# JanEGerken/HEAL-SWIN

Hardware: AMD Instinct MI355X
Metric: images/sec fwd+bwd, HEAL-SWIN nside=256 seg, batch=8 at 1/2/4/8 MI355X (higher is better)
Workload: dtype bf16

## Files before the change

### heal_swin_amd/csrc/expand_ln_head.hip

```cpp
#include "ln_head_device.h"
#include "hs_depth_loss.h"

#pragma clang fp contract(off)
#include "hs_depth_target.h"
#include "hs_depth_metrics.h"
#pragma clang fp contract(fast)

namespace hs {
namespace {

constexpr int kP = 4;
constexpr int kRowB = 256;
constexpr int kPatchRow = 128;

constexpr int kHistBins = kKP * kKP;

__device__ __forceinline__ int argmax_merge(float best, int arg, float ob, int oa) {
    const bool n0 = best != best, n1 = ob != ob;
    const int lower = arg < oa ? arg : oa;
    if (n0 || n1) return n0 && n1 ? lower : (n0 ? arg : oa);
    return best > ob ? arg : (ob > best ? oa : lower);
}

struct TailLane {
    float num = 0.f, den = 0.f;
    uint32_t pred4 = 0;
    uint32_t bad_rows = 0;
    uint32_t* hist = nullptr;
    float4 m4, lv4;
    double dsum[depth_metrics::kNSums];
};

struct TailCe {
    const uint8_t* labels;
    const float* class_w;
    float* loss_part;
    int n_classes;
    __device__ __forceinline__ bool has_loss() const { return labels != nullptr; }
    __device__ __forceinline__ bool ce_row(TailLane& st, const f32x16& lg, const float (&bk)[8], int64_t orow, bool live, int half,
                                           float (&v)[8], int& yl) const {
        if (!labels) return false;
        float m = -INFINITY;
#pragma unroll
        for (int r = 0; r < 8; ++r) {
            v[r] = lg[r] + bk[r];
            if (class_natural(r, half) < n_classes) m = fmaxf(m, v[r]);
        }
        m = fmaxf(m, __shfl_xor(m, 32, 64));
        yl = live ? (int)labels[orow] : 255;
        float ssum = 0.f, pick = 0.f;
#pragma unroll
        for (int r = 0; r < 8; ++r) {
            const int cls = class_natural(r, half);
            if (cls < n_classes) ssum += __builtin_amdgcn_exp2f((v[r] - m) * kLog2e);
            pick = cls == yl ? v[r] : pick;
        }
        ssum += __shfl_xor(ssum, 32, 64);
        pick += __shfl_xor(pick, 32, 64);
        const float wy = yl < n_classes ? (class_w ? class_w[yl] : 1.f) : 0.f;
        if (half == 0) {
            st.num = fmaf(wy, m + __builtin_amdgcn_logf(ssum) * kLn2 - pick, st.num);
            st.den += wy;
        }
        return true;
    }
    __device__ __forceinline__ void row(TailLane& st, const f32x16& lg, const float (&bk)[8], int64_t orow, int, bool live,
                                        int lane) const {
        float v[8];
        int yl;
        ce_row(st, lg, bk, orow, live, lane >> 5, v, yl);
    }
};

struct TailCeStep : TailCe {
    uint8_t* preds;
    unsigned long long* conf;
    unsigned long long* bad;
    __device__ __forceinline__ bool has_loss() const { return true; }
    __device__ __forceinline__ void row(TailLane& st, const f32x16& lg, const float (&bk)[8], int64_t orow, int p, bool live,
                                        int lane) const {
        const int half = lane >> 5;
        float v[8];
        int yl;
        if (!ce_row(st, lg, bk, orow, live, half, v, yl)) return;
        float best = -INFINITY;
        int arg = 4 * half < n_classes ? 4 * half : 64;
#pragma unroll
        for (int r = 0; r < 8; ++r) {
            const int cls = class_natural(r, half);
            if (cls < n_classes && !(best != best) && (v[r] > best || v[r] != v[r])) {
                best = v[r];
                arg = cls;
            }
        }
        const int pred = argmax_merge(best, arg, __shfl_xor(best, 32, 64), __shfl_xor(arg, 32, 64));
        st.pred4 |= (uint32_t)pred << (8 * p);
        if (conf) {
            const bool mine = live && half == 0;
            const int bin = mine && yl < n_classes ? yl * n_classes + pred : -1;
            st.bad_rows += (uint32_t)__popcll(__ballot(mine && yl >= n_classes));
            const int lead = __builtin_amdgcn_readfirstlane(bin);
            const unsigned long long same = __ballot(bin == lead);
            if (bin == lead) {
                if (lead >= 0 && lane == __ffsll((long long)same) - 1) atomicAdd(&st.hist[lead], (uint32_t)__popcll(same));
            } else if (bin >= 0) {
                atomicAdd(&st.hist[bin], 1u);
            }
        }
    }
};

struct TailDepth {
    const float* target;
    float* loss_part;
    int kind;
    float delta;
    __device__ __forceinline__ bool has_loss() const { return true; }
    __device__ __forceinline__ float depth_row(TailLane& st, const f32x16& lg, const float (&bk)[8], int64_t orow, bool live,
                                               int half) const {
        const float t = live && half == 0 ? target[orow] : INFINITY;
        if (depth_keep(t)) {
            st.num += depth_term(kind, delta, lg[0] + bk[0], lg[1] + bk[1], t);
            st.den += 1.f;
        }
        return t;
    }
    __device__ __forceinline__ void row(TailLane& st, const f32x16& lg, const float (&bk)[8], int64_t orow, int, bool live,
                                        int lane) const {
        depth_row(st, lg, bk, orow, live, lane >> 5);
    }
};

struct TailDepthStep : TailDepth {
    int n_out;
    TargetOp inv;
    depth_metrics::Rule rule;
    double* partial;
    float* preds;
    float* logvar_out;
    int64_t rows;
    __device__ __forceinline__ void row(TailLane& st, const f32x16& lg, const float (&bk)[8], int64_t orow, int p, bool live,
                                        int lane) const {
        const int half = lane >> 5;
        const float p0 = lg[0] + bk[0], p1 = lg[1] + bk[1], t = depth_row(st, lg, bk, orow, live, half);
        if (partial || preds) {
#pragma clang fp contract(off)
            const float m = target_op(p0, inv);
            if (partial && live && half == 0)
                depth_metrics::accumulate<float, float>(st.dsum, rule, m, target_op(t, inv), [&] { return p1; });
            st.m4.x = p == 0 ? m : st.m4.x;
            st.m4.y = p == 1 ? m : st.m4.y;
            st.m4.z = p == 2 ? m : st.m4.z;
            st.m4.w = p == 3 ? m : st.m4.w;
        }
        st.lv4.x = p == 0 ? p1 : st.lv4.x;
        st.lv4.y = p == 1 ? p1 : st.lv4.y;
        st.lv4.z = p == 2 ? p1 : st.lv4.z;
        st.lv4.w = p == 3 ? p1 : st.lv4.w;
    }
};

template <int NB, typename Loss>
__global__ void __launch_bounds__(256, 1) expand_ln_head_fwd_kernel(const uint16_t* __restrict__ xn, const uint16_t* __restrict__ xn_lo,
                                                                    const uint16_t* __restrict__ wexp,
                                                                    const uint16_t* __restrict__ wfold, const float* __restrict__ bvec,
                                                                    uint16_t* __restrict__ y, float* __restrict__ logits,
                                                                    float* __restrict__ mean_out, float* __restrict__ rstd_out,
                                                                    int64_t tokens, Loss ce) {
    constexpr bool kStep = std::is_same<Loss, TailCeStep>::value, kDStep = std::is_same<Loss, TailDepthStep>::value;
    constexpr int C = 32 * NB, KS = 2 * NB, NCH = C / 8;
    extern __shared__ __attribute__((aligned(16))) unsigned char smem[];
    unsigned char* wl = smem;
    unsigned char* patch = smem + kP * C * kRowB + (threadIdx.x >> 6) * (32 * kPatchRow);
    const int tid = threadIdx.x, lane = tid & 63, l31 = lane & 31, half = lane >> 5;

    for (int q = tid; q < kP * C * NCH; q += 256) {
        const int row = q / NCH, ch = q % NCH;
        *(uint4*)(wl + row * kRowB + ((ch ^ (row & 15)) << 4)) = *(const uint4*)(wexp + (int64_t)row * C + ch * 8);
    }
    bf16x8 wfa[NB][2], wfl[NB][2];
#pragma unroll
    for (int ct = 0; ct < NB; ++ct)
#pragma unroll
        for (int j = 0; j < 2; ++j) {
            const uint16_t* src = wfold + l31 * C + 32 * ct + 16 * j + 4 * half;
            const uint2 a = *(const uint2*)src, b = *(const uint2*)(src + 8);
            wfa[ct][j] = __builtin_bit_cast(bf16x8, make_uint4(a.x, a.y, b.x, b.y));
            const uint2 al = *(const uint2*)(src + 32 * C), bl = *(const uint2*)(src + 32 * C + 8);
            wfl[ct][j] = __builtin_bit_cast(bf16x8, make_uint4(al.x, al.y, bl.x, bl.y));
        }
    float bk[8];
    load_head_bias(bvec, half, bk);
    uint32_t* hist = (uint32_t*)(smem + kP * C * kRowB + 4 * 32 * kPatchRow);
    TailLane st;
    st.hist = hist + (tid >> 6) * kHistBins;
    if constexpr (kStep) {
        for (int j = tid; j < 4 * kHistBins; j += 256) hist[j] = 0;
    }
    if constexpr (kDStep) {
#pragma unroll
        for (int k = 0; k < depth_metrics::kNSums; ++k) st.dsum[k] = 0.0;
    }
    __syncthreads();

    const int sx = l31 & 15;
    const int64_t wave = (int64_t)blockIdx.x * 4 + (tid >> 6), nwaves = (int64_t)gridDim.x * 4;
    for (int64_t tok0 = wave * 32; tok0 < tokens; tok0 += nwaves * 32) {
        const int64_t tok = tok0 + l31;
        const bool live = tok < tokens;
        bf16x8 xb[KS];
#pragma unroll
        for (int ks = 0; ks < KS; ++ks) {
            const uint4 v = live ? *(const uint4*)(xn + tok * C + 16 * ks + 8 * half) : make_uint4(0, 0, 0, 0);
            xb[ks] = __builtin_bit_cast(bf16x8, v);
        }
        st.pred4 = 0;
        st.m4 = st.lv4 = make_float4(0.f, 0.f, 0.f, 0.f);
#pragma unroll 1
        for (int p = 0; p < kP; ++p) {
            f32x16 acc[NB];
#pragma unroll
            for (int ct = 0; ct < NB; ++ct)
#pragma unroll
                for (int r = 0; r < 16; ++r) acc[ct][r] = 0.f;
            const unsigned char* wrow = wl + (p * C + l31) * kRowB;
#pragma unroll
            for (int ks = 0; ks < KS; ++ks) {
                const int co = ((2 * ks + half) ^ sx) << 4;
#pragma unroll
                for (int ct = 0; ct < NB; ++ct) {
                    const bf16x8 a = *(const bf16x8*)(wrow + ct * 32 * kRowB + co);
                    acc[ct] = __builtin_amdgcn_mfma_f32_32x32x16_bf16(a, xb[ks], acc[ct], 0, 0, 0);
                }
            }
            if (xn_lo) {
#pragma unroll
                for (int ks = 0; ks < KS; ++ks) {
                    const uint4 v = live ? *(const uint4*)(xn_lo + tok * C + 16 * ks + 8 * half) : make_uint4(0, 0, 0, 0);
                    const int co = ((2 * ks + half) ^ sx) << 4;
#pragma unroll
                    for (int ct = 0; ct < NB; ++ct) {
                        const bf16x8 a = *(const bf16x8*)(wrow + ct * 32 * kRowB + co);
                        acc[ct] = __builtin_amdgcn_mfma_f32_32x32x16_bf16(a, __builtin_bit_cast(bf16x8, v), acc[ct], 0, 0, 0);
                    }
                }
            }
            const int64_t orow = tok * kP + p;
            if (y) {
#pragma unroll
                for (int pr = 0; pr < (NB + 1) / 2; ++pr) {
#pragma unroll
                    for (int t = 0; t < 2; ++t) {
                        const int ct = 2 * pr + t;
                        if (ct < NB) {
#pragma unroll
                            for (int g = 0; g < 4; ++g) {
                                const int chunk = 4 * t + g;
                                *(uint2*)(patch + l31 * kPatchRow + ((chunk ^ (l31 & 7)) << 4) + 8 * half) =
                                    make_uint2(pack_bf16x2(acc[ct][4 * g], acc[ct][4 * g + 1]), pack_bf16x2(acc[ct][4 * g + 2], acc[ct][4 * g + 3]));
                            }
                        }
                    }
                    __builtin_amdgcn_fence(__ATOMIC_RELEASE, "wavefront");
                    __builtin_amdgcn_wave_barrier();
                    constexpr int kChunksLast = (NB % 2) ? 4 : 8;
                    const int nchunks = (2 * pr + 1 < NB) ? 8 : kChunksLast;
#pragma unroll
                    for (int i = 0; i < 4; ++i) {
                        const int q = lane + 64 * i, row = q >> 3, chunk = q & 7;
                        const uint4 v = *(const uint4*)(patch + row * kPatchRow + ((chunk ^ (row & 7)) << 4));
                        if (chunk < nchunks && tok0 + row < tokens)
                            *(uint4*)(y + ((tok0 + row) * kP + p) * C + 64 * pr + chunk * 8) = v;
                    }
                    __builtin_amdgcn_fence(__ATOMIC_ACQUIRE, "wavefront");
                    __builtin_amdgcn_wave_barrier();
                }
            }
            float mean, rstd;
            row_stats<16>(acc, mean, rstd);
            f32x16 lg;
#pragma unroll
            for (int r = 0; r < 16; ++r) lg[r] = 0.f;
#pragma unroll
            for (int ct = 0; ct < NB; ++ct)
#pragma unroll
                for (int j = 0; j < 2; ++j) {
                    float xh[8];
#pragma unroll
                    for (int i = 0; i < 8; ++i) xh[i] = acc[ct][8 * j + i] * rstd;
                    lg = head_step<3>(lg, xh, wfa[ct][j], wfl[ct][j]);
                }
            ce.row(st, lg, bk, orow, p, live, lane);
            if (live) {
                if (logits) {
                    *(float4*)(logits + orow * kKP + 4 * half) = make_float4(lg[0] + bk[0], lg[1] + bk[1], lg[2] + bk[2], lg[3] + bk[3]);
                    *(float4*)(logits + orow * kKP + 8 + 4 * half) = make_float4(lg[4] + bk[4], lg[5] + bk[5], lg[6] + bk[6], lg[7] + bk[7]);
                }
                if (half == 0 && mean_out) {
                    mean_out[orow] = mean;
                    rstd_out[orow] = rstd;
                }
            }
        }
        if constexpr (kStep) {
            if (ce.preds && live && half == 0) *(uint32_t*)(ce.preds + tok * kP) = st.pred4;
        }
        if constexpr (kDStep) {
            if (live && half == 0) {
                if (ce.preds) *(float4*)(ce.preds + tok * kP) = st.m4;
                float* lv = ce.preds ? (ce.n_out > 1 ? ce.preds + ce.rows : nullptr) : ce.logvar_out;
                if (lv) *(float4*)(lv + tok * kP) = st.lv4;
            }
        }
    }
    if constexpr (kDStep) {
        if (ce.partial) {
            constexpr int NS = depth_metrics::kNSums;
            static_assert(NS * 256 * sizeof(double) <= kP * 64 * kRowB + 4 * 32 * kPatchRow, "lane sums must fit the LDS at C = 64");
            double* red = (double*)smem;
            __syncthreads();
#pragma unroll
            for (int k = 0; k < NS; ++k) red[k * 256 + tid] = st.dsum[k];
            __syncthreads();
            for (int h = 128; h > 0; h >>= 1) {
                for (int q = tid; q < NS * h; q += 256) {
                    const int k = q / h, j = q - k * h;
                    red[k * 256 + j] += red[k * 256 + j + h];
                }
                __syncthreads();
            }
            if (tid < NS) ce.partial[(int64_t)blockIdx.x * NS + tid] = red[tid * 256];
        }
    }
    if constexpr (kStep) {
        if (ce.conf) {
            __syncthreads();
            const int bins = ce.n_classes * ce.n_classes;
            if (tid < bins) {
                const uint32_t n = hist[tid] + hist[kHistBins + tid] + hist[2 * kHistBins + tid] + hist[3 * kHistBins + tid];
                if (n) atomicAdd(&ce.conf[tid], (unsigned long long)n);
            }
            if (lane == 0 && st.bad_rows) atomicAdd(&ce.bad[0], (unsigned long long)st.bad_rows);
        }
    }
    if (ce.has_loss()) {
        const float n = wave_sum(st.num), d = wave_sum(st.den);
        if (lane == 0) {
            ce.loss_part[2 * wave] = n;
            ce.loss_part[2 * wave + 1] = d;
        }
    }
}

}
}

extern "C" {

int hs_expand_ln_head_supported(int width, int children, int n_classes, int dtype) {
    return dtype == HS_BF16 && children == hs::kP && width % 32 == 0 && width >= 64 && width <= 128 && n_classes >= 1 && n_classes <= 16;
}

extern "C++" {
namespace {
template <typename Loss>
int launch_expand_ln_head(const void* xn, const void* xn_lo, const void* wexp, const void* wfold, const float* bvec, void* y, float* logits,
                          float* mean, float* rstd, int64_t tokens, int width, int children, int dtype, void* stream, Loss ce,
                          const char* who) {
    using namespace hs;
    HS_CHECK_ARG(xn && wexp && wfold && bvec, "%s: null pointer", who);
    HS_CHECK_ARG(tokens > 0, "%s: bad shape", who);
    HS_CHECK_ARG((y == nullptr) == (mean == nullptr) && (mean == nullptr) == (rstd == nullptr),
                 "%s: y, mean and rstd (what the backward needs) go together", who);
    if (!hs_expand_ln_head_supported(width, children, 1, dtype))
        return fail(HS_ERR_UNSUPPORTED, "%s: bf16, 4 children, C in {64, 96, 128} (got C = %d, children %d): the expand "
                    "weight must fit the LDS", who, width, children);
    HS_CHECK_ALIGNED(who, 16, xn, xn_lo, wexp, wfold, bvec, y);
    constexpr bool kStep = std::is_same<Loss, TailCeStep>::value;
    const size_t smem = (size_t)kP * width * kRowB + 4 * 32 * kPatchRow + (kStep ? 4 * kHistBins * sizeof(uint32_t) : 0);
    HS_CHECK_ARG(smem <= 160 * 1024, "%s: %zu bytes of LDS", who, smem);
    const dim3 grid((unsigned)hs_expand_ln_head_blocks(tokens)), block(256);
    if constexpr (kStep) {
        const int64_t groups = (tokens + 31) / 32, waves = (int64_t)grid.x * 4;
        HS_CHECK_ARG((groups + waves - 1) / waves < (1ll << 25), "%s: %lld tokens on %lld waves overflow the 32-bit histogram bins", who,
                     (long long)tokens, (long long)waves);
    }
    return with_width_blocks<4>(width, [&](auto nb) {
        auto kern = expand_ln_head_fwd_kernel<decltype(nb)::value, Loss>;
        static bool configured = false;
        if (!configured) {
            HS_HIP_CHECK(hipFuncSetAttribute((const void*)kern, hipFuncAttributeMaxDynamicSharedMemorySize, (int)smem));
            configured = true;
        }
        hipLaunchKernelGGL(kern, grid, block, smem, (hipStream_t)stream, (const uint16_t*)xn, (const uint16_t*)xn_lo,
                           (const uint16_t*)wexp, (const uint16_t*)wfold, bvec, (uint16_t*)y, logits, mean, rstd, tokens, ce);
        HS_LAUNCH_CHECK("expand_ln_head_fwd");
        return (int)HS_OK;
    });
}
int check_ce_loss(const char* who, const void* labels, const void* loss_partials, int n_classes) {
    HS_CHECK_ARG(labels && loss_partials, "%s: null pointer", who);
    return hs::check_class_count(who, n_classes);
}
int check_depth_loss(const char* who, const void* target, const void* loss_partials, int kind, float huber_delta, int n_out) {
    HS_CHECK_ARG(target && loss_partials, "%s: null pointer", who);
    return hs::check_depth_head(who, kind, huber_delta, n_out);
}
}
}

int64_t hs_expand_ln_head_blocks(int64_t tokens) {
    int64_t blocks = (tokens + 127) / 128;
    const int cus = hs::usable_cus();
    if (blocks > cus) blocks = cus;
    return blocks < 1 ? 1 : blocks;
}

int hs_expand_ln_head_fwd(const void* xn, const void* xn_lo, const void* wexp, const void* wfold, const float* bvec, void* y, float* logits,
                          float* mean, float* rstd, int64_t tokens, int width, int children, int dtype, void* stream) {
    HS_CHECK_ARG(logits, "hs_expand_ln_head_fwd: null pointer");
    return launch_expand_ln_head(xn, xn_lo, wexp, wfold, bvec, y, logits, mean, rstd, tokens, width, children, dtype, stream,
                                 hs::TailCe{nullptr, nullptr, nullptr, 0}, "hs_expand_ln_head_fwd");
}

int hs_expand_ln_head_ce_fwd(const void* xn, const void* xn_lo, const void* wexp, const void* wfold, const float* bvec, const uint8_t* labels,
                             const float* class_weights, int n_classes, void* y, float* logits, float* mean, float* rstd,
                             float* loss_partials, int64_t tokens, int width, int children, int dtype, void* stream) {
    if (int e = check_ce_loss("hs_expand_ln_head_ce_fwd", labels, loss_partials, n_classes)) return e;
    return launch_expand_ln_head(xn, xn_lo, wexp, wfold, bvec, y, logits, mean, rstd, tokens, width, children, dtype, stream,
                                 hs::TailCe{labels, class_weights, loss_partials, n_classes}, "hs_expand_ln_head_ce_fwd");
}

int hs_expand_ln_head_ce_step_fwd(const void* xn, const void* xn_lo, const void* wexp, const void* wfold, const float* bvec,
                                  const uint8_t* labels, const float* class_weights, int n_classes, void* y, float* logits, float* mean,
                                  float* rstd, float* loss_partials, uint8_t* preds, int64_t* confmat, int64_t* bad, int64_t tokens,
                                  int width, int children, int dtype, void* stream) {
    const char* who = "hs_expand_ln_head_ce_step_fwd";
    if (int e = check_ce_loss(who, labels, loss_partials, n_classes)) return e;
    HS_CHECK_ARG(!confmat || bad, "%s: confmat needs bad (the counter of labels >= n_classes)", who);
    HS_CHECK_ARG(((uintptr_t)preds & 3) == 0, "%s: preds must be 4-byte aligned", who);
    return launch_expand_ln_head(xn, xn_lo, wexp, wfold, bvec, y, logits, mean, rstd, tokens, width, children, dtype, stream,
                                 hs::TailCeStep{{labels, class_weights, loss_partials, n_classes}, preds, (unsigned long long*)confmat,
                                                (unsigned long long*)bad}, who);
}

int hs_expand_ln_head_depth_step_fwd(const void* xn, const void* xn_lo, const void* wexp, const void* wfold, const float* bvec,
                                     const float* target, int kind, float huber_delta, int n_out, void* y, float* logits, float* mean,
                                     float* rstd, float* loss_partials, int flags, int transform, float shift, float scale, int use_logvar,
                                     double total_mean, const float* ranges, int n_ranges, double* metric_partials, double* metric_state,
                                     float* preds, float* logvar_out, int64_t tokens, int width, int children, int dtype, void* stream) {
    const char* who = "hs_expand_ln_head_depth_step_fwd";
    if (int e = check_depth_loss(who, target, loss_partials, kind, huber_delta, n_out)) return e;
    HS_CHECK_ARG(transform == HS_DT_NONE || transform == HS_DT_LOG || transform == HS_DT_INV, "%s: transform %d", who, transform);
    HS_CHECK_ARG((flags & ~(HS_DT_AFFINE | HS_DT_INVERSE)) == 0, "%s: flags %d (HS_DT_AFFINE or 0: the inverse chain is applied)", who, flags);
    HS_CHECK_ARG((metric_partials == nullptr) == (metric_state == nullptr), "%s: metric_partials and metric_state go together", who);
    HS_CHECK_ARG(n_out == 2 || !(logvar_out || (use_logvar && metric_state)), "%s: the log variance needs a two-channel head", who);
    hs::TailDepthStep st{{target, loss_partials, kind, huber_delta}, n_out, hs::TargetOp{flags | HS_DT_INVERSE, transform, shift, scale},
                         {}, metric_partials, preds, logvar_out, tokens * hs::kP};
    if (int e = hs::depth_metrics::fill_rule(st.rule, use_logvar, total_mean, ranges, n_ranges)) return e;
    HS_CHECK_ALIGNED(who, 16, preds, logvar_out);
    HS_CHECK_ALIGNED(who, 8, metric_partials, metric_state);
    HS_CHECK_ALIGNED(who, 4, target, loss_partials);
    if (int e = launch_expand_ln_head(xn, xn_lo, wexp, wfold, bvec, y, logits, mean, rstd, tokens, width, children, dtype, stream, st, who))
        return e;
    if (metric_state) {
        hipLaunchKernelGGL(hs::depth_metrics::reduce_kernel, dim3(1), dim3(hs::depth_metrics::kThreads), 0, (hipStream_t)stream,
                           metric_partials, (int)hs_expand_ln_head_blocks(tokens), metric_state);
        HS_LAUNCH_CHECK("expand_ln_head_depth_step_reduce");
    }
    return HS_OK;
}

int hs_expand_ln_head_depth_fwd(const void* xn, const void* xn_lo, const void* wexp, const void* wfold, const float* bvec, const float* target,
                                int kind, float huber_delta, int n_out, void* y, float* logits, float* mean, float* rstd, float* loss_partials,
                                int64_t tokens, int width, int children, int dtype, void* stream) {
    if (int e = check_depth_loss("hs_expand_ln_head_depth_fwd", target, loss_partials, kind, huber_delta, n_out)) return e;
    return launch_expand_ln_head(xn, xn_lo, wexp, wfold, bvec, y, logits, mean, rstd, tokens, width, children, dtype, stream,
                                 hs::TailDepth{target, loss_partials, kind, huber_delta}, "hs_expand_ln_head_depth_fwd");
}

}
```

### heal_swin_amd/csrc/ln_head.hip

```cpp
#include "ln_head_device.h"
#include "hs_depth_loss.h"

namespace hs {
namespace {

template <int NB, bool F32OUT>
__global__ void __launch_bounds__(256) ln_head_fwd_kernel(const uint16_t* __restrict__ y, const uint16_t* __restrict__ wfold,
                                                          const float* __restrict__ bvec, void* __restrict__ logits_v,
                                                          float* __restrict__ mean_out, float* __restrict__ rstd_out, int64_t rows) {
    constexpr int C = NB * 32, NS = NB * 2;
    const int lane = threadIdx.x & 63, l31 = lane & 31, half = lane >> 5;
    const int64_t wave = (int64_t)blockIdx.x * 4 + (threadIdx.x >> 6), nwaves = (int64_t)gridDim.x * 4;
    bf16x8 wa[NS];
#pragma unroll
    for (int s = 0; s < NS; ++s) wa[s] = *(const bf16x8*)(wfold + l31 * C + 16 * s + 8 * half);
    float bk[8];
    load_head_bias(bvec, half, bk);
    for (int64_t row0 = wave * 32; row0 < rows; row0 += nwaves * 32) {
        const int64_t row = row0 + l31;
        const bool live = row < rows;
        float x[NS][8];
#pragma unroll
        for (int s = 0; s < NS; ++s) {
            const uint4 v = live ? *(const uint4*)(y + row * C + 16 * s + 8 * half) : make_uint4(0, 0, 0, 0);
            unpack8(v, x[s]);
        }
        float mean, rstd;
        row_stats<8>(x, mean, rstd);
        f32x16 acc;
#pragma unroll
        for (int r = 0; r < 16; ++r) acc[r] = 0.f;
#pragma unroll
        for (int s = 0; s < NS; ++s) {
#pragma unroll
            for (int j = 0; j < 8; ++j) x[s][j] *= rstd;
            acc = head_step<F32OUT ? 2 : 1>(acc, x[s], wa[s], wa[s]);
        }
        if (live) {
            float o[8];
#pragma unroll
            for (int r = 0; r < 8; ++r) o[r] = acc[r] + bk[r];
            if constexpr (F32OUT) {
                float* logits = (float*)logits_v;
                *(float4*)(logits + row * kKP + 4 * half) = make_float4(o[0], o[1], o[2], o[3]);
                *(float4*)(logits + row * kKP + 8 + 4 * half) = make_float4(o[4], o[5], o[6], o[7]);
            } else {
                uint16_t* logits = (uint16_t*)logits_v;
                const uint4 ob = pack8(o);
                *(uint2*)(logits + row * kKP + 4 * half) = make_uint2(ob.x, ob.y);
                *(uint2*)(logits + row * kKP + 8 + 4 * half) = make_uint2(ob.z, ob.w);
            }
            if (half == 0) {
                mean_out[row] = mean;
                rstd_out[row] = rstd;
            }
        }
    }
}

template <typename T>
struct BwdRows {
    static constexpr bool kFused = false;
    const T* dlogits;
    __device__ __forceinline__ uint4 load(int64_t row, int half, float (&d)[8]) const {
        if constexpr (std::is_same<T, float>::value) {
            const float4 a = *(const float4*)(dlogits + row * kKP + 8 * half);
            const float4 b = *(const float4*)(dlogits + row * kKP + 8 * half + 4);
            d[0] = a.x; d[1] = a.y; d[2] = a.z; d[3] = a.w; d[4] = b.x; d[5] = b.y; d[6] = b.z; d[7] = b.w;
            return pack8(d);
        } else {
            const uint4 dl = *(const uint4*)(dlogits + row * kKP + 8 * half);
            unpack8(dl, d);
            return dl;
        }
    }
};
struct BwdFused {
    static constexpr bool kFused = true;
    const uint16_t* wfold;
    const float* bvec;
    const float* scale;
};
struct BwdCe : BwdFused {
    const uint8_t* labels;
    const float* class_w;
    int n_classes;
    __device__ __forceinline__ int target(int64_t row, bool live, int) const { return live ? (int)labels[row] : 255; }
    __device__ __forceinline__ void grad(const f32x16& lg, const float (&bk)[8], int yl, int half, float s, float (&d)[8]) const {
        float m = -INFINITY;
#pragma unroll
        for (int r = 0; r < 8; ++r) {
            d[r] = lg[r] + bk[r];
            if (class_exchanged(r, half) < n_classes) m = fmaxf(m, d[r]);
        }
        m = fmaxf(m, __shfl_xor(m, 32, 64));
        float ssum = 0.f;
#pragma unroll
        for (int r = 0; r < 8; ++r) {
            d[r] = class_exchanged(r, half) < n_classes ? __builtin_amdgcn_exp2f((d[r] - m) * kLog2e) : 0.f;
            ssum += d[r];
        }
        ssum += __shfl_xor(ssum, 32, 64);
        const float wy = yl < n_classes ? (class_w ? class_w[yl] : 1.f) : 0.f;
        const float coef = s * wy, pinv = 1.f / ssum;
#pragma unroll
        for (int r = 0; r < 8; ++r) d[r] = coef * (d[r] * pinv - (class_exchanged(r, half) == yl ? 1.f : 0.f));
    }
};
struct BwdDepth : BwdFused {
    const float* target_rows;
    int kind;
    float delta;
    __device__ __forceinline__ float target(int64_t row, bool live, int half) const {
        return live && half == 0 ? target_rows[row] : INFINITY;
    }
    __device__ __forceinline__ void grad(const f32x16& lg, const float (&bk)[8], float tgt, int, float s, float (&d)[8]) const {
#pragma unroll
        for (int r = 0; r < 8; ++r) d[r] = 0.f;
        if (depth_keep(tgt)) depth_grad(kind, delta, lg[0] + bk[0], lg[1] + bk[1], tgt, s, &d[0], &d[1]);
    }
};

template <int NB, typename Src>
__global__ void __launch_bounds__(256) ln_head_bwd_kernel(const uint16_t* __restrict__ y, const float* __restrict__ mean_in,
                                                          const float* __restrict__ rstd_in, const Src src,
                                                          const uint16_t* __restrict__ afold, uint16_t* __restrict__ dy,
                                                          uint16_t* __restrict__ dprime, float* __restrict__ part, int64_t rows) {
    constexpr int C = NB * 32, NS = NB * 2;
    const int lane = threadIdx.x & 63, l31 = lane & 31, half = lane >> 5;
    const int64_t wave = (int64_t)blockIdx.x * 4 + (threadIdx.x >> 6), nwaves = (int64_t)gridDim.x * 4;
    [[maybe_unused]] bf16x8 wa[NS], wl[NS];
    [[maybe_unused]] float bk[8], scale = 0.f;
    if constexpr (Src::kFused) {
#pragma unroll
        for (int s = 0; s < NS; ++s) {
            wa[s] = *(const bf16x8*)(src.wfold + l31 * C + 16 * s + 8 * half);
            wl[s] = *(const bf16x8*)(src.wfold + (32 + l31) * C + 16 * s + 8 * half);
        }
        load_head_bias(src.bvec, half, bk);
        scale = src.scale[0];
    }
    bf16x8 aa[NB];
    {
        const int hh = (l31 >> 2) & 1, j4 = l31 & 3, q = l31 >> 3;
        const int c_in = 16 * (q >> 1) + 8 * hh + j4 + 4 * (q & 1);
#pragma unroll
        for (int i = 0; i < NB; ++i) aa[i] = *(const bf16x8*)(afold + (32 * i + c_in) * kKP + 8 * half);
    }
    float uacc[8], tacc[8];
#pragma unroll
    for (int j = 0; j < 8; ++j) uacc[j] = tacc[j] = 0.f;
    const float inv_c = 1.f / (float)C;
    for (int64_t row0 = wave * 32; row0 < rows; row0 += nwaves * 32) {
        const int64_t row = row0 + l31;
        const bool live = row < rows;
        const float mean = live ? mean_in[row] : 0.f, rstd = live ? rstd_in[row] : 0.f;
        uint4 dl = make_uint4(0, 0, 0, 0);
        float d[8] = {0.f, 0.f, 0.f, 0.f, 0.f, 0.f, 0.f, 0.f};
        float xh[NS][8];
        if constexpr (!Src::kFused) {
            if (live) dl = src.load(row, half, d);
        }
        uint4 v[NS];
#pragma unroll
        for (int s = 0; s < NS; ++s) v[s] = live ? *(const uint4*)(y + row * C + 16 * s + 8 * half) : make_uint4(0, 0, 0, 0);
        if constexpr (Src::kFused) {
            const auto tgt = src.target(row, live, half);
            f32x16 lg;
#pragma unroll
            for (int r = 0; r < 16; ++r) lg[r] = 0.f;
#pragma unroll
            for (int s = 0; s < NS; ++s) {
                unpack8(v[s], xh[s]);
#pragma unroll
                for (int j = 0; j < 8; ++j) xh[s][j] = (xh[s][j] - mean) * rstd;
                lg = head_step<3>(lg, xh[s], wa[s], wl[s]);
            }
            src.grad(lg, bk, tgt, half, scale, d);
            dl = pack8(d);
        }
        f32x16 g[NB];
#pragma unroll
        for (int i = 0; i < NB; ++i) {
#pragma unroll
            for (int r = 0; r < 16; ++r) g[i][r] = 0.f;
            g[i] = __builtin_amdgcn_mfma_f32_32x32x16_bf16(aa[i], __builtin_bit_cast(bf16x8, dl), g[i], 0, 0, 0);
        }
        {
            float dp[8];
#pragma unroll
            for (int j = 0; j < 8; ++j) dp[j] = d[j] * rstd;
            const uint4 pk = pack8(dp);
            float dr[8];
            unpack8(pk, dr);
#pragma unroll
            for (int j = 0; j < 8; ++j) {
                uacc[j] += d[j];
                tacc[j] = fmaf(dr[j], mean, tacc[j]);
            }
            if (live) *(uint4*)(dprime + row * kKP + 8 * half) = pk;
        }
        float s1 = 0.f, s2 = 0.f;
#pragma unroll
        for (int s = 0; s < NS; ++s) {
            if constexpr (!Src::kFused) unpack8(v[s], xh[s]);
#pragma unroll
            for (int j = 0; j < 8; ++j) {
                if constexpr (!Src::kFused) xh[s][j] = (xh[s][j] - mean) * rstd;
                const float gv = g[s >> 1][8 * (s & 1) + j];
                s1 += gv;
                s2 = fmaf(gv, xh[s][j], s2);
            }
        }
        s1 += __shfl_xor(s1, 32, 64);
        s2 += __shfl_xor(s2, 32, 64);
        const float m1 = s1 * inv_c, m2 = s2 * inv_c;
#pragma unroll
        for (int s = 0; s < NS; ++s) {
            float o[8];
#pragma unroll
            for (int j = 0; j < 8; ++j) o[j] = rstd * (g[s >> 1][8 * (s & 1) + j] - m1 - xh[s][j] * m2);
            if (live) *(uint4*)(dy + row * C + 16 * s + 8 * half) = pack8(o);
        }
    }
#pragma unroll
    for (int j = 0; j < 8; ++j) {
#pragma unroll
        for (int off = 1; off < 32; off <<= 1) {
            uacc[j] += __shfl_xor(uacc[j], off, 64);
            tacc[j] += __shfl_xor(tacc[j], off, 64);
        }
    }
    if (l31 == 0) {
#pragma unroll
        for (int j = 0; j < 8; ++j) {
            part[wave * 32 + 8 * half + j] = uacc[j];
            part[wave * 32 + 16 + 8 * half + j] = tacc[j];
        }
    }
}

int grid_for(int64_t rows) {
    int64_t b = (rows + 127) / 128;
    if (b > 256 * 8) b = 256 * 8;
    return (int)(b < 1 ? 1 : b);
}

template <typename... P>
uintptr_t address_bits(P... p) {
    return (((uintptr_t)p) | ... | (uintptr_t)0);
}

int check_ln_head_args(const char* who, bool all, uintptr_t vec16, int64_t rows) {
    HS_CHECK_ARG(all, "%s: null pointer", who);
    HS_CHECK_ALIGNED(who, 16, vec16);
    HS_CHECK_ARG(rows > 0, "%s: bad shape", who);
    return HS_OK;
}
int check_ln_head_width(const char* who, int width, int n_out, int dtype, int max_width) {
    if (!hs_ln_head_supported(width, n_out, dtype) || width > max_width)
        return fail(HS_ERR_UNSUPPORTED, "%s: bf16 rows of 64..%d (multiple of 32) columns only", who, max_width);
    return HS_OK;
}
int check_logits_dtype(const char* who, int logits_dtype) {
    HS_CHECK_ARG(logits_dtype == HS_BF16 || logits_dtype == HS_F32, "%s: logits_dtype must be HS_BF16 or HS_F32", who);
    return HS_OK;
}

template <int MAX_NB, typename Src>
int launch_ln_head_bwd(const char* who, const void* y, const float* mean, const float* rstd, const Src& src, const void* afold,
                       void* dy, void* dprime, float* partials, int64_t rows, int width, void* stream) {
    return with_width_blocks<MAX_NB>(width, [&](auto nb) {
        hipLaunchKernelGGL((ln_head_bwd_kernel<decltype(nb)::value, Src>), dim3(grid_for(rows)), dim3(256), 0, (hipStream_t)stream,
                           (const uint16_t*)y, mean, rstd, src, (const uint16_t*)afold, (uint16_t*)dy, (uint16_t*)dprime, partials,
                           rows);
        HS_LAUNCH_CHECK("ln_head_bwd");
        return (int)HS_OK;
    });
}

}
}

extern "C" {

int hs_ln_head_supported(int width, int n_classes, int dtype) {
    return dtype == HS_BF16 && width % 32 == 0 && width >= 64 && width <= 256 && n_classes >= 1 && n_classes <= 16;
}

int64_t hs_ln_head_partials(int64_t rows) { return rows > 0 ? (int64_t)hs::grid_for(rows) * 4 : 0; }

int hs_ln_head_fwd(const void* y, const void* wfold, const float* bvec, void* logits, float* mean, float* rstd, int64_t rows,
                   int width, int dtype, int logits_dtype, void* stream) {
    using namespace hs;
    const char* who = "hs_ln_head_fwd";
    const bool all = y && wfold && bvec && logits && mean && rstd;
    if (int e = check_ln_head_args(who, all, address_bits(y, wfold, bvec), rows)) return e;
    if (int e = check_logits_dtype(who, logits_dtype)) return e;
    if (int e = check_ln_head_width(who, width, 1, dtype, 256)) return e;
    return with_width_blocks<8>(width, [&](auto nb) {
        auto kern = logits_dtype == HS_F32 ? ln_head_fwd_kernel<decltype(nb)::value, true> : ln_head_fwd_kernel<decltype(nb)::value, false>;
        hipLaunchKernelGGL(kern, dim3(grid_for(rows)), dim3(256), 0, (hipStream_t)stream, (const uint16_t*)y, (const uint16_t*)wfold,
                           bvec, logits, mean, rstd, rows);
        HS_LAUNCH_CHECK("ln_head_fwd");
        return (int)HS_OK;
    });
}

int hs_ln_head_bwd(const void* y, const float* mean, const float* rstd, const void* dlogits, const void* afold, void* dy,
                   void* dprime, float* partials, int64_t rows, int width, int dtype, int logits_dtype, void* stream) {
    using namespace hs;
    const char* who = "hs_ln_head_bwd";
    const bool all = y && mean && rstd && dlogits && afold && dy && dprime && partials;
    if (int e = check_ln_head_args(who, all, address_bits(y, afold, dy, dprime), rows)) return e;
    if (int e = check_logits_dtype(who, logits_dtype)) return e;
    if (int e = check_ln_head_width(who, width, 1, dtype, 256)) return e;
    if (logits_dtype == HS_F32)
        return launch_ln_head_bwd<8>(who, y, mean, rstd, BwdRows<float>{(const float*)dlogits}, afold, dy, dprime, partials, rows, width,
                                     stream);
    return launch_ln_head_bwd<8>(who, y, mean, rstd, BwdRows<uint16_t>{(const uint16_t*)dlogits}, afold, dy, dprime, partials, rows,
                                 width, stream);
}

int hs_ln_head_ce_bwd(const void* y, const float* mean, const float* rstd, const uint8_t* labels, const float* class_weights,
                      const float* scale, int n_classes, const void* wfold, const float* bvec, const void* afold, void* dy,
                      void* dprime, float* partials, int64_t rows, int width, int dtype, void* stream) {
    using namespace hs;
    const char* who = "hs_ln_head_ce_bwd";
    const bool all = y && mean && rstd && labels && scale && wfold && bvec && afold && dy && dprime && partials;
    if (int e = check_ln_head_args(who, all, address_bits(y, wfold, bvec, afold, dy, dprime), rows)) return e;
    if (int e = check_class_count(who, n_classes)) return e;
    if (int e = check_ln_head_width(who, width, n_classes, dtype, 128)) return e;
    const BwdCe src{{(const uint16_t*)wfold, bvec, scale}, labels, class_weights, n_classes};
    return launch_ln_head_bwd<4>(who, y, mean, rstd, src, afold, dy, dprime, partials, rows, width, stream);
}

int hs_ln_head_depth_bwd(const void* y, const float* mean, const float* rstd, const float* target, int kind, float huber_delta,
                         const float* scale, int n_out, const void* wfold, const float* bvec, const void* afold, void* dy,
                         void* dprime, float* partials, int64_t rows, int width, int dtype, void* stream) {
    using namespace hs;
    const char* who = "hs_ln_head_depth_bwd";
    const bool all = y && mean && rstd && target && scale && wfold && bvec && afold && dy && dprime && partials;
    if (int e = check_ln_head_args(who, all, address_bits(y, wfold, bvec, afold, dy, dprime), rows)) return e;
    if (int e = check_depth_head(who, kind, huber_delta, n_out)) return e;
    if (int e = check_ln_head_width(who, width, n_out, dtype, 128)) return e;
    const BwdDepth src{{(const uint16_t*)wfold, bvec, scale}, target, kind, huber_delta};
    return launch_ln_head_bwd<4>(who, y, mean, rstd, src, afold, dy, dprime, partials, rows, width, stream);
}

}
```

### heal_swin_amd/csrc/ln_head_device.h

```cpp
#pragma once
#include <type_traits>

#include "hs_device.h"

namespace hs {

constexpr float kEps = 1e-5f;
constexpr int kKP = 16;

__device__ __forceinline__ void unpack8(const uint4& v, float* f) {
    const uint32_t w[4] = {v.x, v.y, v.z, v.w};
#pragma unroll
    for (int i = 0; i < 4; ++i) {
        f[2 * i] = bf_lo(w[i]);
        f[2 * i + 1] = bf_hi(w[i]);
    }
}
__device__ __forceinline__ uint4 pack8(const float* f) {
    return make_uint4(pack_bf16x2(f[0], f[1]), pack_bf16x2(f[2], f[3]), pack_bf16x2(f[4], f[5]), pack_bf16x2(f[6], f[7]));
}

__device__ __forceinline__ int class_natural(int r, int half) { return 4 * half + (r & 3) + 8 * (r >> 2); }
__device__ __forceinline__ int class_exchanged(int r, int half) { return 8 * half + r; }

__device__ __forceinline__ void load_head_bias(const float* __restrict__ bvec, int half, float (&bk)[8]) {
#pragma unroll
    for (int r = 0; r < 8; ++r) bk[r] = bvec[class_natural(r, half)];
}

template <int K, int M, typename Regs>
__device__ __forceinline__ void row_stats(Regs (&v)[M], float& mean, float& rstd) {
    constexpr float inv_c = 1.f / (float)(2 * M * K);
    float sum = 0.f;
#pragma unroll
    for (int m = 0; m < M; ++m)
#pragma unroll
        for (int k = 0; k < K; ++k) sum += v[m][k];
    sum += __shfl_xor(sum, 32, 64);
    mean = sum * inv_c;
    float sq = 0.f;
#pragma unroll
    for (int m = 0; m < M; ++m)
#pragma unroll
        for (int k = 0; k < K; ++k) {
            v[m][k] -= mean;
            sq = fmaf(v[m][k], v[m][k], sq);
        }
    sq += __shfl_xor(sq, 32, 64);
    rstd = rsqrtf(sq * inv_c + kEps);
}

template <int TERMS>
__device__ __forceinline__ f32x16 head_step(f32x16 acc, const float (&xh)[8], bf16x8 wa, bf16x8 wl) {
    const uint4 hb = pack8(xh);
    acc = __builtin_amdgcn_mfma_f32_32x32x16_bf16(wa, __builtin_bit_cast(bf16x8, hb), acc, 0, 0, 0);
    if constexpr (TERMS >= 2) {
        float hi[8], lo[8];
        unpack8(hb, hi);
#pragma unroll
        for (int j = 0; j < 8; ++j) lo[j] = xh[j] - hi[j];
        acc = __builtin_amdgcn_mfma_f32_32x32x16_bf16(wa, __builtin_bit_cast(bf16x8, pack8(lo)), acc, 0, 0, 0);
    }
    if constexpr (TERMS >= 3) acc = __builtin_amdgcn_mfma_f32_32x32x16_bf16(wl, __builtin_bit_cast(bf16x8, hb), acc, 0, 0, 0);
    return acc;
}

inline int check_class_count(const char* who, int n_classes) {
    HS_CHECK_ARG(n_classes >= 1 && n_classes <= kKP, "%s: 1..16 classes", who);
    return HS_OK;
}

template <int MAX_NB, class F>
int with_width_blocks(int width, F&& f) {
    switch (width / 32) {
        case 2: return f(std::integral_constant<int, 2>{});
        case 3: return f(std::integral_constant<int, 3>{});
        case 4: return f(std::integral_constant<int, 4>{});
    }
    if constexpr (MAX_NB >= 8) {
        switch (width / 32) {
            case 5: return f(std::integral_constant<int, 5>{});
            case 6: return f(std::integral_constant<int, 6>{});
            case 7: return f(std::integral_constant<int, 7>{});
            case 8: return f(std::integral_constant<int, 8>{});
        }
    }
    return fail(HS_ERR_UNSUPPORTED, "decoder tail: no kernel for %d columns", width);
}

}
```

Baseline: 56.71.

## Prefetch next token group's activations and targets in decoder tail kernels

Both the fused expand-LN-head forward and the LN-head backward kernels now issue global loads for the next grid-stride iteration (activations, lo-part, mean/rstd, labels or depth targets) before computing the current one. Empty asm barriers tie each load's use to a later accumulator value, so the compiler cannot sink the loads and their latency overlaps the MFMA work. Per-class CE weights are preloaded once per lane and fetched with a shuffle instead of a gathered global load. This costs more registers, with some values parked in AGPRs, and is disabled for a few width/loss combinations, presumably where register pressure would hurt occupancy.

New measurement: 56.88 (median of 6 runs). About the same (+0.3%).

```diff
diff --git a/heal_swin_amd/csrc/expand_ln_head.hip b/heal_swin_amd/csrc/expand_ln_head.hip
--- a/heal_swin_amd/csrc/expand_ln_head.hip
+++ b/heal_swin_amd/csrc/expand_ln_head.hip
@@ -14,6 +14,14 @@
 constexpr int kPatchRow = 128;
 
 constexpr int kHistBins = kKP * kKP;
+
+struct Four {
+    float a, b, c, d;
+};
+using hs::arrived;
+__device__ __forceinline__ void arrived(Four& v, float after) {
+    asm volatile("" : "+v"(v.a), "+v"(v.b), "+v"(v.c), "+v"(v.d) : "v"(after));
+}
 
 __device__ __forceinline__ int argmax_merge(float best, int arg, float ob, int oa) {
     const bool n0 = best != best, n1 = ob != ob;
@@ -27,6 +35,7 @@
     uint32_t pred4 = 0;
     uint32_t bad_rows = 0;
     uint32_t* hist = nullptr;
+    float cw = 1.f;
     float4 m4, lv4;
     double dsum[depth_metrics::kNSums];
 };
@@ -37,8 +46,17 @@
     float* loss_part;
     int n_classes;
     __device__ __forceinline__ bool has_loss() const { return labels != nullptr; }
-    __device__ __forceinline__ bool ce_row(TailLane& st, const f32x16& lg, const float (&bk)[8], int64_t orow, bool live, int half,
-                                           float (&v)[8], int& yl) const {
+    __device__ __forceinline__ void init(TailLane& st, int lane) const {
+        if (kPipe && labels) st.cw = lane_class_weight(class_w, n_classes, lane);
+    }
+    __device__ __forceinline__ int fetch(int64_t orow, bool live, int) const { return labels && live ? (int)labels[orow] : 255; }
+    __device__ __forceinline__ uint32_t fetch4(int64_t tok, bool live, int) const {
+        uint32_t w = 0xffffffffu;
+        if (labels && live) __builtin_memcpy(&w, labels + tok * kP, 4);
+        return w;
+    }
+    static __device__ __forceinline__ int pick(uint32_t w, int p) { return (int)((w >> (8 * p)) & 255u); }
+    __device__ __forceinline__ bool ce_row(TailLane& st, const f32x16& lg, const float (&bk)[8], int yl, int half, float (&v)[8]) const {
         if (!labels) return false;
         float m = -INFINITY;
 #pragma unroll
@@ -47,7 +65,6 @@
             if (class_natural(r, half) < n_classes) m = fmaxf(m, v[r]);
         }
         m = fmaxf(m, __shfl_xor(m, 32, 64));
-        yl = live ? (int)labels[orow] : 255;
         float ssum = 0.f, pick = 0.f;
 #pragma unroll
         for (int r = 0; r < 8; ++r) {
@@ -57,18 +74,22 @@
         }
         ssum += __shfl_xor(ssum, 32, 64);
         pick += __shfl_xor(pick, 32, 64);
-        const float wy = yl < n_classes ? (class_w ? class_w[yl] : 1.f) : 0.f;
+        float wy;
+        if constexpr (kPipe) {
+            const float wsh = __shfl(st.cw, yl & 15, 64);
+            wy = yl < n_classes ? wsh : 0.f;
+        } else {
+            wy = yl < n_classes ? (class_w ? class_w[yl] : 1.f) : 0.f;
+        }
         if (half == 0) {
             st.num = fmaf(wy, m + __builtin_amdgcn_logf(ssum) * kLn2 - pick, st.num);
             st.den += wy;
         }
         return true;
     }
-    __device__ __forceinline__ void row(TailLane& st, const f32x16& lg, const float (&bk)[8], int64_t orow, int, bool live,
-                                        int lane) const {
+    __device__ __forceinline__ void row(TailLane& st, const f32x16& lg, const float (&bk)[8], int yl, int, bool, int lane) const {
         float v[8];
-        int yl;
-        ce_row(st, lg, bk, orow, live, lane >> 5, v, yl);
+        ce_row(st, lg, bk, yl, lane >> 5, v);
     }
 };
 
@@ -77,12 +98,11 @@
     unsigned long long* conf;
     unsigned long long* bad;
     __device__ __forceinline__ bool has_loss() const { return true; }
-    __device__ __forceinline__ void row(TailLane& st, const f32x16& lg, const float (&bk)[8], int64_t orow, int p, bool live,
+    __device__ __forceinline__ void row(TailLane& st, const f32x16& lg, const float (&bk)[8], int yl, int p, bool live,
                                         int lane) const {
         const int half = lane >> 5;
         float v[8];
-        int yl;
-        if (!ce_row(st, lg, bk, orow, live, half, v, yl)) return;
+        if (!ce_row(st, lg, bk, yl, half, v)) return;
         float best = -INFINITY;
         int arg = 4 * half < n_classes ? 4 * half : 64;
 #pragma unroll
@@ -116,18 +136,25 @@
     int kind;
     float delta;
     __device__ __forceinline__ bool has_loss() const { return true; }
-    __device__ __forceinline__ float depth_row(TailLane& st, const f32x16& lg, const float (&bk)[8], int64_t orow, bool live,
-                                               int half) const {
-        const float t = live && half == 0 ? target[orow] : INFINITY;
+    __device__ __forceinline__ void init(TailLane&, int) const {}
+    __device__ __forceinline__ float fetch(int64_t orow, bool live, int half) const {
+        return live && half == 0 ? target[orow] : INFINITY;
+    }
+    __device__ __forceinline__ Four fetch4(int64_t tok, bool live, int half) const {
+        Four w = {INFINITY, INFINITY, INFINITY, INFINITY};
+        if (live && half == 0) __builtin_memcpy(&w, target + tok * kP, 16);
+        return w;
+    }
+    static __device__ __forceinline__ float pick(const Four& w, int p) { return p == 0 ? w.a : p == 1 ? w.b : p == 2 ? w.c : w.d; }
+    __device__ __forceinline__ float depth_row(TailLane& st, const f32x16& lg, const float (&bk)[8], float t) const {
         if (depth_keep(t)) {
             st.num += depth_term(kind, delta, lg[0] + bk[0], lg[1] + bk[1], t);
             st.den += 1.f;
         }
         return t;
     }
-    __device__ __forceinline__ void row(TailLane& st, const f32x16& lg, const float (&bk)[8], int64_t orow, int, bool live,
-                                        int lane) const {
-        depth_row(st, lg, bk, orow, live, lane >> 5);
+    __device__ __forceinline__ void row(TailLane& st, const f32x16& lg, const float (&bk)[8], float t, int, bool, int) const {
+        depth_row(st, lg, bk, t);
     }
 };
 
@@ -139,10 +166,10 @@
     float* preds;
     float* logvar_out;
     int64_t rows;
-    __device__ __forceinline__ void row(TailLane& st, const f32x16& lg, const float (&bk)[8], int64_t orow, int p, bool live,
+    __device__ __forceinline__ void row(TailLane& st, const f32x16& lg, const float (&bk)[8], float tgt, int p, bool live,
                                         int lane) const {
         const int half = lane >> 5;
-        const float p0 = lg[0] + bk[0], p1 = lg[1] + bk[1], t = depth_row(st, lg, bk, orow, live, half);
+        const float p0 = lg[0] + bk[0], p1 = lg[1] + bk[1], t = depth_row(st, lg, bk, tgt);
         if (partial || preds) {
 #pragma clang fp contract(off)
             const float m = target_op(p0, inv);
@@ -169,6 +196,7 @@
                                                                     int64_t tokens, Loss ce) {
     constexpr bool kStep = std::is_same<Loss, TailCeStep>::value, kDStep = std::is_same<Loss, TailDepthStep>::value;
     constexpr int C = 32 * NB, KS = 2 * NB, NCH = C / 8;
+    constexpr bool kAhead = kPipe && !(kDStep && NB == 4);
     extern __shared__ __attribute__((aligned(16))) unsigned char smem[];
     unsigned char* wl = smem;
     unsigned char* patch = smem + kP * C * kRowB + (threadIdx.x >> 6) * (32 * kPatchRow);
@@ -194,6 +222,7 @@
     uint32_t* hist = (uint32_t*)(smem + kP * C * kRowB + 4 * 32 * kPatchRow);
     TailLane st;
     st.hist = hist + (tid >> 6) * kHistBins;
+    ce.init(st, lane);
     if constexpr (kStep) {
         for (int j = tid; j < 4 * kHistBins; j += 256) hist[j] = 0;
     }
@@ -205,19 +234,56 @@
 
     const int sx = l31 & 15;
     const int64_t wave = (int64_t)blockIdx.x * 4 + (tid >> 6), nwaves = (int64_t)gridDim.x * 4;
+    using Want = decltype(ce.fetch4((int64_t)0, false, 0));
+    struct Group {
+        bf16x8 hi[KS], lo[KS];
+        Want want;
+    };
+    auto request = [&](int64_t t0, Group& g) __attribute__((always_inline)) {
+        const int64_t t = t0 + l31;
+        const bool lv = t < tokens;
+#pragma unroll
+        for (int ks = 0; ks < KS; ++ks) {
+            const uint4 v = lv ? *(const uint4*)(xn + t * C + 16 * ks + 8 * half) : make_uint4(0, 0, 0, 0);
+            g.hi[ks] = __builtin_bit_cast(bf16x8, v);
+        }
+#pragma unroll
+        for (int ks = 0; ks < KS; ++ks) {
+            const uint4 v = xn_lo && lv ? *(const uint4*)(xn_lo + t * C + 16 * ks + 8 * half) : make_uint4(0, 0, 0, 0);
+            g.lo[ks] = __builtin_bit_cast(bf16x8, v);
+        }
+        g.want = ce.fetch4(t, lv, half);
+    };
+    auto settle = [&](Group& g, float after) __attribute__((always_inline)) {
+#pragma unroll
+        for (int ks = 0; ks < KS; ++ks) {
+            arrived(g.hi[ks], after);
+            arrived(g.lo[ks], after);
+        }
+        arrived(g.want, after);
+    };
+    [[maybe_unused]] Group cur, nxt;
+    if constexpr (kAhead) {
+        request(wave * 32, cur);
+        settle(cur, 0.f);
+    }
     for (int64_t tok0 = wave * 32; tok0 < tokens; tok0 += nwaves * 32) {
         const int64_t tok = tok0 + l31;
         const bool live = tok < tokens;
-        bf16x8 xb[KS];
-#pragma unroll
-        for (int ks = 0; ks < KS; ++ks) {
-            const uint4 v = live ? *(const uint4*)(xn + tok * C + 16 * ks + 8 * half) : make_uint4(0, 0, 0, 0);
-            xb[ks] = __builtin_bit_cast(bf16x8, v);
-        }
+        if constexpr (kAhead) {
+            request(tok0 + nwaves * 32, nxt);
+        } else {
+#pragma unroll
+            for (int ks = 0; ks < KS; ++ks) {
+                const uint4 v = live ? *(const uint4*)(xn + tok * C + 16 * ks + 8 * half) : make_uint4(0, 0, 0, 0);
+                cur.hi[ks] = __builtin_bit_cast(bf16x8, v);
+            }
+        }
+        const bf16x8(&xb)[KS] = cur.hi;
+        const Want want = kAhead ? cur.want : Want{};
         st.pred4 = 0;
         st.m4 = st.lv4 = make_float4(0.f, 0.f, 0.f, 0.f);
-#pragma unroll 1
-        for (int p = 0; p < kP; ++p) {
+        auto child = [&](const int p, auto first) __attribute__((always_inline)) {
             f32x16 acc[NB];
 #pragma unroll
             for (int ct = 0; ct < NB; ++ct)
@@ -236,14 +302,23 @@
             if (xn_lo) {
 #pragma unroll
                 for (int ks = 0; ks < KS; ++ks) {
-                    const uint4 v = live ? *(const uint4*)(xn_lo + tok * C + 16 * ks + 8 * half) : make_uint4(0, 0, 0, 0);
+                    bf16x8 b;
+                    if constexpr (kAhead) {
+                        b = cur.lo[ks];
+                    } else {
+                        const uint4 v = live ? *(const uint4*)(xn_lo + tok * C + 16 * ks + 8 * half) : make_uint4(0, 0, 0, 0);
+                        b = __builtin_bit_cast(bf16x8, v);
+                    }
                     const int co = ((2 * ks + half) ^ sx) << 4;
 #pragma unroll
                     for (int ct = 0; ct < NB; ++ct) {
                         const bf16x8 a = *(const bf16x8*)(wrow + ct * 32 * kRowB + co);
-                        acc[ct] = __builtin_amdgcn_mfma_f32_32x32x16_bf16(a, __builtin_bit_cast(bf16x8, v), acc[ct], 0, 0, 0);
+                        acc[ct] = __builtin_amdgcn_mfma_f32_32x32x16_bf16(a, b, acc[ct], 0, 0, 0);
                     }
                 }
+            }
+            if constexpr (kAhead) {
+                if constexpr (decltype(first)::value) settle(nxt, acc[NB - 1][15]);
             }
             const int64_t orow = tok * kP + p;
             if (y) {
@@ -290,7 +365,7 @@
                     for (int i = 0; i < 8; ++i) xh[i] = acc[ct][8 * j + i] * rstd;
                     lg = head_step<3>(lg, xh, wfa[ct][j], wfl[ct][j]);
                 }
-            ce.row(st, lg, bk, orow, p, live, lane);
+            ce.row(st, lg, bk, kAhead ? ce.pick(want, p) : ce.fetch(orow, live, half), p, live, lane);
             if (live) {
                 if (logits) {
                     *(float4*)(logits + orow * kKP + 4 * half) = make_float4(lg[0] + bk[0], lg[1] + bk[1], lg[2] + bk[2], lg[3] + bk[3]);
@@ -301,6 +376,14 @@
                     rstd_out[orow] = rstd;
                 }
             }
+        };
+        if constexpr (kAhead) {
+            child(0, std::true_type{});
+#pragma unroll 1
+            for (int p = 1; p < kP; ++p) child(p, std::false_type{});
+        } else {
+#pragma unroll 1
+            for (int p = 0; p < kP; ++p) child(p, std::false_type{});
         }
         if constexpr (kStep) {
             if (ce.preds && live && half == 0) *(uint32_t*)(ce.preds + tok * kP) = st.pred4;
@@ -311,6 +394,14 @@
                 float* lv = ce.preds ? (ce.n_out > 1 ? ce.preds + ce.rows : nullptr) : ce.logvar_out;
                 if (lv) *(float4*)(lv + tok * kP) = st.lv4;
             }
+        }
+        if constexpr (kAhead) {
+#pragma unroll
+            for (int ks = 0; ks < KS; ++ks) {
+                cur.hi[ks] = nxt.hi[ks];
+                cur.lo[ks] = nxt.lo[ks];
+            }
+            cur.want = nxt.want;
         }
     }
     if constexpr (kDStep) {
diff --git a/heal_swin_amd/csrc/ln_head.hip b/heal_swin_amd/csrc/ln_head.hip
--- a/heal_swin_amd/csrc/ln_head.hip
+++ b/heal_swin_amd/csrc/ln_head.hip
@@ -58,18 +58,37 @@
     }
 }
 
+__device__ __forceinline__ uint4 as_uint4(const u32x4& v) { return make_uint4(v[0], v[1], v[2], v[3]); }
+
 template <typename T>
 struct BwdRows {
     static constexpr bool kFused = false;
     const T* dlogits;
-    __device__ __forceinline__ uint4 load(int64_t row, int half, float (&d)[8]) const {
+    struct Raw {
+        u32x4 a, b;
+    };
+    __device__ __forceinline__ Raw target(int64_t row, bool live, int half) const {
+        Raw r = {u32x4{0, 0, 0, 0}, u32x4{0, 0, 0, 0}};
+        if (live) {
+            r.a = *(const u32x4*)(dlogits + row * kKP + 8 * half);
+            if constexpr (std::is_same<T, float>::value) r.b = *(const u32x4*)(dlogits + row * kKP + 8 * half + 4);
+        }
+        return r;
+    }
+    static __device__ __forceinline__ void settle(Raw& r, float after) {
+        arrived(r.a, after);
+        if constexpr (std::is_same<T, float>::value) arrived(r.b, after);
+    }
+    static __device__ __forceinline__ uint4 take(const Raw& r, float (&d)[8]) {
         if constexpr (std::is_same<T, float>::value) {
-            const float4 a = *(const float4*)(dlogits + row * kKP + 8 * half);
-            const float4 b = *(const float4*)(dlogits + row * kKP + 8 * half + 4);
-            d[0] = a.x; d[1] = a.y; d[2] = a.z; d[3] = a.w; d[4] = b.x; d[5] = b.y; d[6] = b.z; d[7] = b.w;
+#pragma unroll
+            for (int j = 0; j < 4; ++j) {
+                d[j] = __uint_as_float(r.a[j]);
+                d[4 + j] = __uint_as_float(r.b[j]);
+            }
             return pack8(d);
         } else {
-            const uint4 dl = *(const uint4*)(dlogits + row * kKP + 8 * half);
+            const uint4 dl = as_uint4(r.a);
             unpack8(dl, d);
             return dl;
         }
@@ -80,13 +99,18 @@
     const uint16_t* wfold;
     const float* bvec;
     const float* scale;
+    template <typename T>
+    static __device__ __forceinline__ void settle(T& t, float after) {
+        arrived(t, after);
+    }
 };
 struct BwdCe : BwdFused {
     const uint8_t* labels;
     const float* class_w;
     int n_classes;
     __device__ __forceinline__ int target(int64_t row, bool live, int) const { return live ? (int)labels[row] : 255; }
-    __device__ __forceinline__ void grad(const f32x16& lg, const float (&bk)[8], int yl, int half, float s, float (&d)[8]) const {
+    __device__ __forceinline__ float lane_weight(int lane) const { return lane_class_weight(class_w, n_classes, lane); }
+    __device__ __forceinline__ void grad(const f32x16& lg, const float (&bk)[8], int yl, int half, float s, float cwl, float (&d)[8]) const {
         float m = -INFINITY;
 #pragma unroll
         for (int r = 0; r < 8; ++r) {
@@ -101,7 +125,13 @@
             ssum += d[r];
         }
         ssum += __shfl_xor(ssum, 32, 64);
-        const float wy = yl < n_classes ? (class_w ? class_w[yl] : 1.f) : 0.f;
+        float wy;
+        if constexpr (kPipe) {
+            const float wsh = __shfl(cwl, yl & 15, 64);
+            wy = yl < n_classes ? wsh : 0.f;
+        } else {
+            wy = yl < n_classes ? (class_w ? class_w[yl] : 1.f) : 0.f;
+        }
         const float coef = s * wy, pinv = 1.f / ssum;
 #pragma unroll
         for (int r = 0; r < 8; ++r) d[r] = coef * (d[r] * pinv - (class_exchanged(r, half) == yl ? 1.f : 0.f));
@@ -114,7 +144,8 @@
     __device__ __forceinline__ float target(int64_t row, bool live, int half) const {
         return live && half == 0 ? target_rows[row] : INFINITY;
     }
-    __device__ __forceinline__ void grad(const f32x16& lg, const float (&bk)[8], float tgt, int, float s, float (&d)[8]) const {
+    __device__ __forceinline__ float lane_weight(int) const { return 1.f; }
+    __device__ __forceinline__ void grad(const f32x16& lg, const float (&bk)[8], float tgt, int, float s, float, float (&d)[8]) const {
 #pragma unroll
         for (int r = 0; r < 8; ++r) d[r] = 0.f;
         if (depth_keep(tgt)) depth_grad(kind, delta, lg[0] + bk[0], lg[1] + bk[1], tgt, s, &d[0], &d[1]);
@@ -127,11 +158,13 @@
                                                           const uint16_t* __restrict__ afold, uint16_t* __restrict__ dy,
                                                           uint16_t* __restrict__ dprime, float* __restrict__ part, int64_t rows) {
     constexpr int C = NB * 32, NS = NB * 2;
+    constexpr bool kAhead = kPipe && NB <= 4 && !(std::is_same<Src, BwdDepth>::value && NB == 3);
     const int lane = threadIdx.x & 63, l31 = lane & 31, half = lane >> 5;
     const int64_t wave = (int64_t)blockIdx.x * 4 + (threadIdx.x >> 6), nwaves = (int64_t)gridDim.x * 4;
     [[maybe_unused]] bf16x8 wa[NS], wl[NS];
-    [[maybe_unused]] float bk[8], scale = 0.f;
+    [[maybe_unused]] float bk[8], scale = 0.f, cwl = 1.f;
     if constexpr (Src::kFused) {
+        cwl = src.lane_weight(lane);
 #pragma unroll
         for (int s = 0; s < NS; ++s) {
             wa[s] = *(const bf16x8*)(src.wfold + l31 * C + 16 * s + 8 * half);
@@ -151,21 +184,51 @@
 #pragma unroll
     for (int j = 0; j < 8; ++j) uacc[j] = tacc[j] = 0.f;
     const float inv_c = 1.f / (float)C;
+    using Want = decltype(src.target((int64_t)0, false, 0));
+    struct Step {
+        u32x4 v[NS];
+        float mean, rstd;
+        Want want;
+    };
+    auto request = [&](int64_t r0, Step& t) __attribute__((always_inline)) {
+        const int64_t r = r0 + l31;
+        const bool lv = r < rows;
+        t.mean = lv ? mean_in[r] : 0.f;
+        t.rstd = lv ? rstd_in[r] : 0.f;
+#pragma unroll
+        for (int s = 0; s < NS; ++s) t.v[s] = lv ? *(const u32x4*)(y + r * C + 16 * s + 8 * half) : u32x4{0, 0, 0, 0};
+        t.want = src.target(r, lv, half);
+    };
+    auto settle = [&](Step& t, float after) __attribute__((always_inline)) {
+        arrived(t.mean, after);
+        arrived(t.rstd, after);
+        Src::settle(t.want, after);
+#pragma unroll
+        for (int s = 0; s < NS; ++s) arrived_parked(t.v[s], after);
+    };
+    [[maybe_unused]] Step cur, nxt;
+    if constexpr (kAhead) {
+        request(wave * 32, cur);
+        settle(cur, 0.f);
+    }
     for (int64_t row0 = wave * 32; row0 < rows; row0 += nwaves * 32) {
         const int64_t row = row0 + l31;
         const bool live = row < rows;
-        const float mean = live ? mean_in[row] : 0.f, rstd = live ? rstd_in[row] : 0.f;
+        if constexpr (kAhead) {
+            request(row0 + nwaves * 32, nxt);
+        } else {
+            request(row0, cur);
+        }
+        const float mean = cur.mean, rstd = cur.rstd;
+        uint4 v[NS];
+#pragma unroll
+        for (int s = 0; s < NS; ++s) v[s] = as_uint4(cur.v[s]);
         uint4 dl = make_uint4(0, 0, 0, 0);
         float d[8] = {0.f, 0.f, 0.f, 0.f, 0.f, 0.f, 0.f, 0.f};
         float xh[NS][8];
-        if constexpr (!Src::kFused) {
-            if (live) dl = src.load(row, half, d);
-        }
-        uint4 v[NS];
-#pragma unroll
-        for (int s = 0; s < NS; ++s) v[s] = live ? *(const uint4*)(y + row * C + 16 * s + 8 * half) : make_uint4(0, 0, 0, 0);
+        if constexpr (!Src::kFused) dl = Src::take(cur.want, d);
         if constexpr (Src::kFused) {
-            const auto tgt = src.target(row, live, half);
+            const auto tgt = cur.want;
             f32x16 lg;
 #pragma unroll
             for (int r = 0; r < 16; ++r) lg[r] = 0.f;
@@ -176,7 +239,7 @@
                 for (int j = 0; j < 8; ++j) xh[s][j] = (xh[s][j] - mean) * rstd;
                 lg = head_step<3>(lg, xh[s], wa[s], wl[s]);
             }
-            src.grad(lg, bk, tgt, half, scale, d);
+            src.grad(lg, bk, tgt, half, scale, cwl, d);
             dl = pack8(d);
         }
         f32x16 g[NB];
@@ -198,6 +261,7 @@
                 uacc[j] += d[j];
                 tacc[j] = fmaf(dr[j], mean, tacc[j]);
             }
+            if constexpr (kAhead) settle(nxt, __uint_as_float(pk.x));
             if (live) *(uint4*)(dprime + row * kKP + 8 * half) = pk;
         }
         float s1 = 0.f, s2 = 0.f;
@@ -221,6 +285,13 @@
 #pragma unroll
             for (int j = 0; j < 8; ++j) o[j] = rstd * (g[s >> 1][8 * (s & 1) + j] - m1 - xh[s][j] * m2);
             if (live) *(uint4*)(dy + row * C + 16 * s + 8 * half) = pack8(o);
+        }
+        if constexpr (kAhead) {
+#pragma unroll
+            for (int s = 0; s < NS; ++s) cur.v[s] = nxt.v[s];
+            cur.mean = nxt.mean;
+            cur.rstd = nxt.rstd;
+            cur.want = nxt.want;
         }
     }
 #pragma unroll
diff --git a/heal_swin_amd/csrc/ln_head_device.h b/heal_swin_amd/csrc/ln_head_device.h
--- a/heal_swin_amd/csrc/ln_head_device.h
+++ b/heal_swin_amd/csrc/ln_head_device.h
@@ -7,6 +7,28 @@
 
 constexpr float kEps = 1e-5f;
 constexpr int kKP = 16;
+
+#ifndef HS_TAIL_PIPELINE
+#define HS_TAIL_PIPELINE 1
+#endif
+constexpr bool kPipe = HS_TAIL_PIPELINE != 0;
+
+template <typename T>
+__device__ __forceinline__ void arrived(T& v, float after) {
+    asm volatile("" : "+v"(v) : "v"(after));
+}
+__device__ __forceinline__ void arrived(bf16x8& v, float after) {
+    u32x4 w = __builtin_bit_cast(u32x4, v);
+    asm volatile("" : "+v"(w) : "v"(after));
+    v = __builtin_bit_cast(bf16x8, w);
+}
+template <typename T>
+__device__ __forceinline__ void arrived_parked(T& v, float after) {
+    asm volatile("" : "+a"(v) : "v"(after));
+}
+__device__ __forceinline__ float lane_class_weight(const float* __restrict__ class_w, int n_classes, int lane) {
+    return class_w ? ((lane & 15) < n_classes ? class_w[lane & 15] : 0.f) : 1.f;
+}
 
 __device__ __forceinline__ void unpack8(const uint4& v, float* f) {
     const uint32_t w[4] = {v.x, v.y, v.z, v.w};
```
